# EtherealEngine/Universal-Volumetric

Hardware: AMD Instinct MI355X
Metric: frames/s encode, 100k-vert mesh + 2048^2 texture (higher is better)
Workload: dtype u8/int32 (f32 only in the quantiser)

## Files before the change

universal-volumetric_amd/csrc/geo_conn.hpp:

```cpp
__global__ void __launch_bounds__(UVOL_BLOCK) k_face_time(GeoJob *jobs) {
  JOB_OR_RETURN;
  const uint32_t i = blockIdx.x * UVOL_BLOCK + threadIdx.x;
  if (i < (uint32_t)J.nsym) { const int c = J.proc[i]; J.face_time[c / 3] = (int32_t)i; J.tstart[J.nsym - 1 - (int)i] = code_of_corner(c); }
  if (i < (uint32_t)J.ninit) { const int c = J.initc[i]; J.face_time[c / 3] = -(int32_t)i - 2; J.tstart[J.nsym + (int)i] = code_of_corner(c); }
}
__device__ __forceinline__ int att_vertex(const GeoJob &J, int slot, int c);
__device__ __forceinline__ int rec_vertex_field(const GeoJob &J, int t, int c, int r8) {
  if (r8 == 2) { const uint32_t *q = reinterpret_cast<const uint32_t *>(J.rec[1 + t]) + 4 * (size_t)(c / 3); return (int)((uint32_t)((((uint64_t)q[1] << 32) | q[0]) >> (21 * (c % 3))) & 0x1fffffu); }
  const size_t code = (size_t)code_of_corner(c);
  return r8 ? (int)((uint32_t)J.rec[1 + t][2 * code] & 0x1fffffu) : J.rec[1 + t][4 * code];
}
__global__ void __launch_bounds__(UVOL_BLOCK) k_v2d(GeoJob *jobs, int r8) {
  GeoJob &J = jobs[blockIdx.y];
  const int t = blockIdx.z;
  const uint32_t i = blockIdx.x * UVOL_BLOCK + threadIdx.x;
  const bool live = J.status == 0 && !(t > 0 && (t - 1 >= J.nad || !J.interior_seams[t - 1]));
  if (blockIdx.x * UVOL_BLOCK >= (live ? J.ne[t] : 0u)) return;
  int lo0 = 0x7fffffff, hi0 = -0x7fffffff - 1, lo1 = 0x7fffffff, hi1 = -0x7fffffff - 1;
  int iu = -1;
  if (J.qpos) for (int k = 0; k < J.nad; k++) if (J.att_kind[k] == 0 && (J.interior_seams[k] ? t == 1 + k : t == 0)) iu = k;
  if (i < J.ne[t]) {
    const int c = J.order[t][i];
    int vid, pid = 0;
    if (!J.qpos) vid = rec_vertex_field(J, t, c, r8) >> 1;
// ... 88 lines not shown
        const int v_start = act ? UVOL_ALOAD(&vval[vn_]) : 0;
        int acc = 0;
        for (int k = start; k + 1 < e; k++) {
          const int ka = (int)UVOL_READLANE(va_, k), kn = (int)UVOL_READLANE(vn_, k), kp = (int)UVOL_READLANE(vp_, k);
          const uint32_t kd = UVOL_READLANE(dpk, k);
          const int hit = (vn_ == ka ? (int)(kd & 3u) : 0) + (vn_ == kn ? (int)((kd >> 2) & 3u) : 0) + (vn_ == kp ? (int)(kd >> 4) : 0);
          acc += (int)lane > k ? hit : 0;
        }
        if (act) {
          const int av = v_start - acc;
          if (mi > 0) { const int cv = av < 2 ? 2 : (av > 7 ? 7 : av); J.ctx_of[mi] = (uint8_t)(cv - 2); }
          if (dpk & 3u) UVOL_AADD(&vval[va_], -(int)(dpk & 3u));
          UVOL_AADD(&vval[vn_], -(int)((dpk >> 2) & 3u));
          UVOL_AADD(&vval[vp_], -(int)(dpk >> 4));
        }
        UVOL_WAVE_FENCE();
        UVOL_WAVE_SYNC();
      }
      if (e < cnt) {
        const int i = base + e;
        const int lc = (int)UVOL_READLANE(c_, e);
        const int ia = (int)UVOL_READLANE(va_, e), in_ = (int)UVOL_READLANE(vn_, e), ip = (int)UVOL_READLANE(vp_, e);
        if (lane == 0) {
          const int nx = g_nxt(lc), pv = g_prv(lc);
          const int val_n = UVOL_ALOAD(&vval[in_]), val_p = UVOL_ALOAD(&vval[ip]);
          UVOL_ASTORE(&vval[in_], val_n - 1); UVOL_ASTORE(&vval[ip], val_p - 1);
          int nleft = 0, a = opp[pv];
          while (a >= 0) { if (ftime[a / 3] <= i) break; nleft++; a = opp[g_nxt(a)]; }
          UVOL_ASTORE(&vval[ia], nleft + 1);
          const int newv = nvval; int nright = 0; a = opp[nx];
          while (a >= 0) { if (ftime[a / 3] <= i) break; nright++; c2vm[g_nxt(a)] = newv; a = opp[g_prv(a)]; }
          UVOL_ASTORE(&vval[nvval], nright + 1);
          if (i > 0) { const int cv = val_n < 2 ? 2 : (val_n > 7 ? 7 : val_n); J.ctx_of[i] = (uint8_t)(cv - 2); }
        }
        nvval++;
        UVOL_WAVE_FENCE();
        UVOL_WAVE_SYNC();
        if (mi < nsym && (int)lane > e) { va_ = c2vm[c_]; vn_ = c2vm[g_nxt(c_)]; vp_ = c2vm[g_prv(c_)]; }
      }
      start = e + 1;
    }
  }
}

__global__ void __launch_bounds__(64) k_eb_ctx(GeoJob *jobs) {
  GeoJob &J = jobs[blockIdx.x];
  UVOL_SERIAL_PRIO();
  const uint32_t lane = threadIdx.x;
  const int nsym = J.status == 0 ? J.nsym : 0;
  uint32_t cnt[6] = {0, 0, 0, 0, 0, 0};
  for (int base = 1; base < nsym; base += 64) {
    const int i = base + (int)lane;
    const int cx = i < nsym ? J.ctx_of[i] : 7;
    for (int c = 0; c < 6; c++) cnt[c] += (uint32_t)__popcll(__ballot(cx == c));
  }
  uint32_t base_c[6]; { uint32_t o = 0; for (int c = 0; c < 6; c++) { base_c[c] = o; o += cnt[c]; } }
  uint32_t *all = J.ctx_all;
  const unsigned long long lt = lane == 0 ? 0ull : (~0ull >> (64 - lane));
  for (int base = 1; base < nsym; base += 64) {
    const int i = base + (int)lane;
    const bool in = i < nsym;
    const int cx = in ? J.ctx_of[i] : 7;
    const int ps = in ? J.symb[i - 1] : 0;
    const uint32_t id = ps == 0 ? 0u : (ps == 1 ? 1u : (ps == 3 ? 2u : (ps == 5 ? 3u : 4u)));
    for (int c = 0; c < 6; c++) {
      const unsigned long long m = __ballot(in && cx == c);
      if (in && cx == c) all[base_c[c] + (uint32_t)__popcll(m & lt)] = id;
      base_c[c] += (uint32_t)__popcll(m);
    }
  }
  if (lane == 0 && J.status == 0) for (int c = 0; c < 6; c++) { J.ctx_n[c] = cnt[c]; J.rs[c].n = cnt[c]; J.ctx_sym[c] = all + (base_c[c] - cnt[c]); J.rs[c].syms = J.ctx_sym[c]; }
}

__device__ __forceinline__ bool fseam_bit(const GeoJob &J, int slot, int c) { return (J.fseam[c / 3] >> (3 * slot + c % 3)) & 1u; }
__device__ __forceinline__ int st_opp(const GeoJob &J, int slot, int c) { if (c < 0) return GEO_INV; if (slot >= 0 && fseam_bit(J, slot, c)) return GEO_INV; return J.opp[c]; }
__device__ __forceinline__ int st_swl(const GeoJob &J, int slot, int c) { const int o = st_opp(J, slot, g_nxt(c)); return o < 0 ? GEO_INV : g_nxt(o); }
__device__ __forceinline__ int st_swr(const GeoJob &J, int slot, int c) { const int o = st_opp(J, slot, g_prv(c)); return o < 0 ? GEO_INV : g_prv(o); }
__device__ __forceinline__ bool vseam_bit(const GeoJob &J, int slot, uint32_t v) { return (J.vseam[slot][v >> 5] >> (v & 31)) & 1u; }
__device__ __forceinline__ int att_vertex(const GeoJob &J, int slot, int c) {
  const int v = geo_vt(J)[c];
  return (J.interior_seams[slot] && vseam_bit(J, slot, (uint32_t)v)) ? J.avert[slot][c] : v;
}
__global__ void __launch_bounds__(UVOL_BLOCK) k_seams(GeoJob *jobs) {
  JOB_OR_RETURN;
  const uint32_t f = blockIdx.x * UVOL_BLOCK + threadIdx.x;
  if (f >= J.nf) return;
  const uvol_s3 o3 = *reinterpret_cast<const uvol_s3 *>(J.opp + 3 * (size_t)f);
  const int opp_[3] = { o3.x, o3.y, o3.z };
  uint32_t bits = 0;
  for (int i = 0; i < J.nad; i++) {
    const int32_t *A = J.att_kind[i] == 0 ? J.cu : J.cn;
    const uvol_s3 a3 = *reinterpret_cast<const uvol_s3 *>(A + 3 * (size_t)f);
    const int a[3] = { a3.x, a3.y, a3.z };
    bool any = false;
    for (int k = 0; k < 3; k++) {
      uint32_t sm = 1;
      if (opp_[k] >= 0) {
        const int oo = opp_[k], fo = 3 * (oo / 3), jo = oo - fo;
        const uvol_s3 b3 = *reinterpret_cast<const uvol_s3 *>(A + fo);
        const int b[3] = { b3.x, b3.y, b3.z };
        sm = (a[(k + 1) % 3] != b[(jo + 2) % 3] || a[(k + 2) % 3] != b[(jo + 1) % 3]) ? 1u : 0u;
        if (sm) {
          any = true;
          const uint32_t va = (uint32_t)geo_vt(J)[3 * f + (k + 1) % 3], vb = (uint32_t)geo_vt(J)[3 * f + (k + 2) % 3];
          atomicOr(&J.vseam[i][va >> 5], 1u << (va & 31)); atomicOr(&J.vseam[i][vb >> 5], 1u << (vb & 31));
        }
      }
      bits |= sm << (3 * i + k);
    }
    if (any) J.interior_seams[i] = 1;
  }
  J.fseam[f] = (uint8_t)bits;
}
__global__ void __launch_bounds__(UVOL_BLOCK) k_sb_count(GeoJob *jobs) {
  JOB_OR_RETURN_UNIFORM;
  const uint32_t f = blockIdx.x * UVOL_BLOCK + threadIdx.x;
  uint32_t cnt = 0;
  if (f < J.nf) {
    const int x0 = J.tstart[f], fo = x0 >> 2, r0 = x0 & 3;
    const uvol_s3 o3 = *reinterpret_cast<const uvol_s3 *>(J.opp + 3 * (size_t)fo);
    const int opp_[3] = { o3.x, o3.y, o3.z };
    const uint32_t fs = J.fseam[fo];
    int nb[3];
    for (int k = 0; k < 3; k++) nb[k] = opp_[k] < 0 ? -1 : J.face_time[opp_[k] / 3];
    uint32_t b0 = 0, b1 = 0;
    for (int k = 0; k < 3; k++) {
      const int j = (r0 + k) % 3;
      if (opp_[j] < 0) continue;
      const int t = nb[j], df = t >= 0 ? J.nsym - 1 - t : J.nsym + (-t - 2);
      if ((uint32_t)df <= f) continue;
      b0 |= ((fs >> j) & 1u) << cnt; b1 |= ((fs >> (3 + j)) & 1u) << cnt; cnt++;
    }
    J.sbpack[f] = (uint8_t)(cnt | (b0 << 2) | (b1 << 5));
  }
  const uint32_t tot = block_sum(cnt);
  if (threadIdx.x == 0 && blockIdx.x < uvol_blocks_dev(J.nf)) J.bsum[blockIdx.x] = tot;
}
__global__ void __launch_bounds__(UVOL_BLOCK) k_sb_write(GeoJob *jobs) {
  GeoJob &J = jobs[blockIdx.y];
  const bool ok = J.status == 0;
  const uint32_t nf = ok ? J.nf : 0u, f = blockIdx.x * UVOL_BLOCK + threadIdx.x;
  const uint32_t pk = f < nf ? J.sbpack[f] : 0u, cnt = pk & 3u;
  uint32_t tot;
  const uint32_t pos = block_excl_scan(cnt, &tot) + ((ok && blockIdx.x <= uvol_blocks_dev(J.nf)) ? J.bsum[blockIdx.x] : 0);
  __shared__ uint32_t zc[2];
  if (threadIdx.x < 2) zc[threadIdx.x] = 0;
  __syncthreads();
  if (cnt) for (int i = 0; i < J.nad; i++) {
    const uint32_t b = (pk >> (2 + 3 * i)) & 7u; uint32_t z = 0;
    for (uint32_t k = 0; k < cnt; k++) { const uint8_t sb = (uint8_t)((b >> k) & 1u); J.seam_bits[i][pos + k] = sb; z += sb ? 0u : 1u; }
    if (z) atomicAdd(&zc[i], z);
  }
  __syncthreads();
  if (threadIdx.x < 2 && zc[threadIdx.x]) atomicAdd(&J.rb[1 + threadIdx.x].zeros, zc[threadIdx.x]);
  if (blockIdx.x == 0 && threadIdx.x == 0 && ok) {
    const uint32_t n = J.bsum[uvol_blocks_dev(J.nf)];
    J.n_elig = n; for (int i = 0; i < J.nad; i++) J.rb[1 + i].n = n;
  }
}

__global__ void __launch_bounds__(UVOL_BLOCK) k_aseg_a(GeoJob *jobs) {
  JOB_OR_RETURN;
  const int i = (int)blockIdx.z;
  if (i >= J.nad || !J.interior_seams[i]) return;
  const uint32_t c0 = blockIdx.x * (UVOL_BLOCK * GEO_ILP) + threadIdx.x, nc = J.nc;
  int32_t v[GEO_ILP]; uint32_t w[GEO_ILP];
#pragma unroll
  for (int k = 0; k < GEO_ILP; k++) { const uint32_t c = c0 + k * UVOL_BLOCK; v[k] = c < nc ? geo_vt(J)[c] : 0; }
#pragma unroll
  for (int k = 0; k < GEO_ILP; k++) w[k] = J.vseam[i][(uint32_t)v[k] >> 5];
#pragma unroll
  for (int k = 0; k < GEO_ILP; k++) {
    const uint32_t c = c0 + k * UVOL_BLOCK;
    if (c >= nc || !((w[k] >> ((uint32_t)v[k] & 31)) & 1u)) continue;
    if (fseam_bit(J, i, g_nxt((int)c))) J.avert[i][c] = (int32_t)(J.nverts_t[0] + atomicAdd(&J.nseg[i], 1u));
  }
}
__global__ void __launch_bounds__(UVOL_BLOCK) k_aseg_b(GeoJob *jobs) {
  JOB_OR_RETURN;
  const int i = (int)blockIdx.z;
  if (i >= J.nad || !J.interior_seams[i]) return;
  const uint32_t c0 = blockIdx.x * (UVOL_BLOCK * GEO_ILP) + threadIdx.x, nc = J.nc;
  if (c0 == 0) { const uint32_t tot = J.nverts_t[0] + J.nseg[i]; J.nverts_t[2 + i] = tot; if (tot > J.ecap) J.status = GEO_E_WS_OVERFLOW; }
  uint32_t v[GEO_ILP], w[GEO_ILP];
#pragma unroll
  for (int k = 0; k < GEO_ILP; k++) { const uint32_t c = c0 + k * UVOL_BLOCK; v[k] = c < nc ? (uint32_t)geo_vt(J)[c] : 0u; }
#pragma unroll
  for (int k = 0; k < GEO_ILP; k++) w[k] = J.vseam[i][v[k] >> 5];
#pragma unroll
  for (int k = 0; k < GEO_ILP; k++) {
    const uint32_t c = c0 + k * UVOL_BLOCK;
    if (c >= nc || !((w[k] >> (v[k] & 31)) & 1u)) continue;
    int l = (int)c; uint32_t guard = 0;
    for (;;) { const int nl = st_swl(J, i, l); if (nl < 0) break; l = nl; if (++guard > nc) { J.status = -22; return; } }
    if (l != (int)c) J.avert[i][c] = J.avert[i][l];
  }
}
```

universal-volumetric_amd/csrc/geo_walk_lds.hpp:

```cpp
__device__ __forceinline__ bool dense_table_live(const GeoJob &J, int which) { const int ai = which >= 2 ? which - 2 : 0; return !(which >= 2 && (ai >= J.nad || !J.interior_seams[ai])); }
__device__ __forceinline__ void pack_face_records(int32_t *rec, uint32_t f, const int vc[3], const int r[3], int r8) {
  if (r8 == 2) {
    uint64_t lo = 0, hi = 0;
    for (int k = 0; k < 3; k++) { lo |= (uint64_t)((uint32_t)vc[k] & 0x1fffffu) << (21 * k); hi |= (uint64_t)((uint32_t)code_of_corner(r[k]) & 0x1fffffu) << (21 * k); }
    reinterpret_cast<uint4 *>(rec)[f] = make_uint4((uint32_t)lo, (uint32_t)(lo >> 32), (uint32_t)hi, (uint32_t)(hi >> 32));
  } else if (r8) {
    uint4 *dst = reinterpret_cast<uint4 *>(rec) + 2 * (size_t)f;
    uint2 q[3];
    for (int k = 0; k < 3; k++) {
      const uint32_t R = (uint32_t)code_of_corner(r[(k + 1) % 3]) & 0x1fffffu, L = (uint32_t)code_of_corner(r[(k + 2) % 3]) & 0x1fffffu;
      q[k] = make_uint2(((uint32_t)vc[k] & 0x1fffffu) | (R << 21), (R >> 11) | (L << 10));
    }
    dst[0] = make_uint4(q[0].x, q[0].y, q[1].x, q[1].y);
    dst[1] = make_uint4(q[2].x, q[2].y, 0u, 0u);
  } else {
    int4 *dst = reinterpret_cast<int4 *>(rec) + 4 * (size_t)f;
    for (int k = 0; k < 3; k++) dst[k] = make_int4(vc[k], code_of_corner(r[(k + 1) % 3]), code_of_corner(r[(k + 2) % 3]), code_of_corner(r[k]));
    dst[3] = make_int4(0, 0, 0, 0);
  }
}
__device__ __forceinline__ void pack_dummy_record(int32_t *rec, uint32_t nf, int r8) { if (r8 == 2) reinterpret_cast<uint4 *>(rec)[nf] = make_uint4(0xffffffffu, 0xffffffffu, 0xffffffffu, 0xffffffffu); }
__global__ void __launch_bounds__(UVOL_BLOCK) k_pack_faces(GeoJob *jobs, int which, int r8) {
  JOB_OR_RETURN;
  const uint32_t f = blockIdx.x * UVOL_BLOCK + threadIdx.x;
  if (f >= J.nf) return;
  const int ai = which >= 2 ? which - 2 : 0;
  if (which >= 2 && (ai >= J.nad || !J.interior_seams[ai])) return;
  if (f == 0) pack_dummy_record(J.rec[which], J.nf, r8);
  const int32_t *opp = which == 0 ? J.opp : J.nopp;
  const uint8_t *seam = which >= 2 ? J.seam[ai] : nullptr;
  const int32_t *vert = which == 0 ? J.vert : (which == 1 ? J.bvert : J.avert[ai]);
  const uint8_t *vopen = J.vopen_d[which];
  int r[3], vc[3];
  for (int k = 0; k < 3; k++) {
    const int c = 3 * (int)f + k;
    r[k] = (seam && seam[c]) ? GEO_INV : opp[c];
    const int v = vert[c];
    vc[k] = (v << 1) | (vopen[v] ? 1 : 0);
  }
  pack_face_records(J.rec[which], f, vc, r, r8);
  if (which == 0) J.face_time[f] = -1;
}
__global__ void __launch_bounds__(UVOL_BLOCK) k_pack0(GeoJob *jobs, int r8) {
  JOB_OR_RETURN;
  const uint32_t f = blockIdx.x * UVOL_BLOCK + threadIdx.x;
  if (f == 0) { const uint32_t tot = J.n_pos + J.extra_v; J.nverts_t[0] = tot; J.nverts_t[1] = tot; if (tot > J.ecap) J.status = GEO_E_WS_OVERFLOW; }
  if (f >= J.nf) return;
  int r[3], vc[3];
  for (int k = 0; k < 3; k++) {
    const int c = 3 * (int)f + k;
    r[k] = J.opp[c];
    const uint32_t v = (uint32_t)geo_vt(J)[c];
    vc[k] = (int)((v << 1) | ((v < J.ecap && J.vopen_d[0][v]) ? 1u : 0u));
  }
  pack_face_records(J.rec[0], f, vc, r, r8);
  if (f == 0) pack_dummy_record(J.rec[0], J.nf, r8);
  J.face_time[f] = -1;
}
__global__ void __launch_bounds__(UVOL_BLOCK) k_pack_tabs(GeoJob *jobs, int r8, int first) {
  JOB_OR_RETURN;
  const int which = first + (int)blockIdx.z;
  const uint32_t f = blockIdx.x * UVOL_BLOCK + threadIdx.x;
  if (f >= J.nf || !dense_table_live(J, which)) return;
  if (f == 0) pack_dummy_record(J.rec[which], J.nf, r8);
  const int ai = which >= 2 ? which - 2 : -1;
  const uint32_t nbase = J.nverts_t[0], fs = ai >= 0 ? (uint32_t)J.fseam[f] >> (3 * ai) : 0u;
  const uvol_s3 o3 = *reinterpret_cast<const uvol_s3 *>(J.opp + 3 * (size_t)f), v3 = *reinterpret_cast<const uvol_s3 *>(geo_vt(J) + 3 * (size_t)f);
  const int oo[3] = { o3.x, o3.y, o3.z }, vv[3] = { v3.x, v3.y, v3.z };
  int r[3], vc[3];
  for (int k = 0; k < 3; k++) {
    r[k] = ((fs >> k) & 1u) ? GEO_INV : oo[k];
    uint32_t v = (uint32_t)vv[k];
    if (ai >= 0 && ((J.vseam[ai][v >> 5] >> (v & 31)) & 1u)) v = (uint32_t)J.avert[ai][3 * f + k];
    vc[k] = (int)((v << 1) | ((v >= nbase || J.vopen_d[0][v]) ? 1u : 0u));
  }
  pack_face_records(J.rec[which], f, vc, r, r8);
}

#ifdef HIPEMU
typedef int4 uvol_i4;
#else
typedef int uvol_i4 __attribute__((ext_vector_type(4)));
#endif
#ifdef HIPEMU
struct uvol_i3 { int x, y, z; };
template <typename P> __device__ __forceinline__ uvol_i3 rec3(P rec, int code) { const uvol_i4 q = rec[code]; uvol_i3 r; r.x = q.x; r.y = q.y; r.z = q.z; return r; }
#else
typedef int uvol_i3 __attribute__((ext_vector_type(3)));
template <typename P> __device__ __forceinline__ uvol_i3 rec3(P rec, int code) { return *(UVOL_G(const uvol_i3))(rec + code); }
#endif
__device__ __forceinline__ uint32_t pword(UVOL_L(uint32_t) w, int k) { return w[k]; }
#ifndef HIPEMU
__device__ __forceinline__ uint32_t pword(UVOL_G(uint32_t) w, int k) { return __hip_atomic_load(&w[k], __ATOMIC_RELAXED, __HIP_MEMORY_SCOPE_WORKGROUP); }
#endif
template <typename P> __device__ __forceinline__ bool pbit_get(P w, int i) { return (pword(w, i >> 5) >> (i & 31)) & 1u; }
template <typename P> __device__ __forceinline__ void pbit_set(P w, int i) { UVOL_OR_NORET(&w[i >> 5], 1u << (i & 31)); }
__device__ __forceinline__ int code_nxt(int x) { return (x & 3) == 2 ? x - 2 : x + 1; }
__device__ __forceinline__ int code_prv(int x) { return (x & 3) == 0 ? x + 2 : x - 1; }
__device__ __forceinline__ int corner_of_code(int x) { return 3 * (x >> 2) + (x & 3); }

#ifdef HIPEMU
struct uvol_u2 { uint32_t x, y; };
#else
typedef uint32_t uvol_u2 __attribute__((ext_vector_type(2)));
#endif
__device__ __forceinline__ void rec8_dec(uint32_t lo, uint32_t hi, int &vi, int &rc, int &lc) {
  vi = (int)(lo & 0x1fffffu);
  rc = (int)(((lo >> 21) | (hi << 11)) << 11) >> 11;
  lc = (int)(hi << 1) >> 11;
}
template <bool R8> struct RecOps;
template <> struct RecOps<false> {
  typedef UVOL_G(const uvol_i4) Ptr; typedef uvol_i3 Pre;
  static __device__ __forceinline__ Ptr ptr(const int32_t *p) { return UVOL_TO_G(const uvol_i4, reinterpret_cast<const uvol_i4 *>(p)); }
  static __device__ __forceinline__ void get(Ptr rec, int code, int &vi, int &rc, int &lc) { const uvol_i4 q = rec[code]; vi = q.x; rc = q.y; lc = q.z; }
  static __device__ __forceinline__ Pre pre(Ptr rec, int code) { return rec3(rec, code); }
  static __device__ __forceinline__ void take(const Pre &p, int &vi, int &rc, int &lc) { vi = UVOL_READFIRST(p.x); const int l_ = UVOL_READFIRST(p.z); rc = UVOL_READFIRST(p.y); lc = l_; }
};
template <> struct RecOps<true> {
  typedef UVOL_G(const uvol_u2) Ptr; typedef uvol_u2 Pre;
  static __device__ __forceinline__ Ptr ptr(const int32_t *p) { return UVOL_TO_G(const uvol_u2, reinterpret_cast<const uvol_u2 *>(p)); }
  static __device__ __forceinline__ void get(Ptr rec, int code, int &vi, int &rc, int &lc) { const uvol_u2 q = rec[code]; rec8_dec(q.x, q.y, vi, rc, lc); }
  static __device__ __forceinline__ Pre pre(Ptr rec, int code) { return rec[code]; }
  static __device__ __forceinline__ void take(const Pre &p, int &vi, int &rc, int &lc) { const uint32_t lo = (uint32_t)UVOL_READFIRST(p.x), hi = (uint32_t)UVOL_READFIRST(p.y); rec8_dec(lo, hi, vi, rc, lc); }
};

#define WALK_STG 256
#define WALK_STG_DWORDS (WALK_STG + WALK_STG / 4)
struct WalkStage {
  UVOL_L(int32_t) w; UVOL_L(uint8_t) b;
  __device__ __forceinline__ void init(UVOL_L(uint32_t) lds) { w = (UVOL_L(int32_t))lds; b = (UVOL_L(uint8_t))(lds + WALK_STG); }
  __device__ __forceinline__ void flush_words(UVOL_G(int32_t) dst, int n) {
    UVOL_G(uvol_i4) d = (UVOL_G(uvol_i4))(dst + (n - WALK_STG)); UVOL_L(const uvol_i4) s = (UVOL_L(const uvol_i4))w;
#pragma unroll 8
    for (int i = 0; i < WALK_STG / 4; i++) d[i] = s[i];
  }
  __device__ __forceinline__ void flush_bytes(UVOL_G(uint8_t) dst, int n) {
    UVOL_G(uvol_i4) d = (UVOL_G(uvol_i4))(dst + (n - WALK_STG)); UVOL_L(const uvol_i4) s = (UVOL_L(const uvol_i4))b;
#pragma unroll 8
    for (int i = 0; i < WALK_STG / 16; i++) d[i] = s[i];
  }
  __device__ __forceinline__ void tail_words(UVOL_G(int32_t) dst, int n) { for (int i = n & ~(WALK_STG - 1); i < n; i++) dst[i] = w[i & (WALK_STG - 1)]; }
  __device__ __forceinline__ void tail_bytes(UVOL_G(uint8_t) dst, int n) { for (int i = n & ~(WALK_STG - 1); i < n; i++) dst[i] = b[i & (WALK_STG - 1)]; }
};
template <bool R8, typename FB, typename VB>
__device__ __forceinline__ void eb_walk_lane0(GeoJob &J, FB fbits, VB vbits, UVOL_L(uint32_t) stg_lds) {
  typedef RecOps<R8> RO;
  const int nf = (int)J.nf;
  const typename RO::Ptr rec = RO::ptr(J.rec[0]);
  UVOL_G(int32_t) proc = UVOL_TO_G(int32_t, J.proc); UVOL_G(int32_t) stack = UVOL_TO_G(int32_t, J.stack);
  UVOL_G(int32_t) initc = UVOL_TO_G(int32_t, J.initc);
  UVOL_G(uint8_t) symb = UVOL_TO_G(uint8_t, J.symb); UVOL_G(uint8_t) start_bits = UVOL_TO_G(uint8_t, J.start_bits);
  const int dz = UVOL_LANE_ZERO();
  WalkStage stg; stg.init(stg_lds);
  int nproc = 0, ninit = 0, nstart = 0, nsplit = 0;
#define W_EMIT(SYM) do { stg.b[nproc & (WALK_STG - 1)] = (uint8_t)(SYM); nproc++; if ((nproc & (WALK_STG - 1)) == 0) { stg.flush_words(proc, nproc); stg.flush_bytes(symb, nproc); } } while (0)
  enum { T_C = 0, T_S = 1, T_L = 3, T_R = 5, T_E = 7 };
  const bool rl = J.relabel != 0; UVOL_G(const int32_t) s_of_o = UVOL_TO_G(const int32_t, J.s_of_o);
  for (int fo = 0; fo < nf; fo++) {
// ... 237 lines not shown
```

universal-volumetric_amd/csrc/geom_encode.hip:

```cpp
#include <chrono>
#include <thread>
#include "uvol_common.hpp"
#include "geom_device.hpp"
#include "uvol_ws.hpp"
#include <algorithm>
#include <map>

#define JOB_OR_RETURN GeoJob &J = jobs[blockIdx.y]; if (J.status != 0) return
#define JOB_OR_RETURN_UNIFORM GeoJob &J = jobs[blockIdx.y]; { __shared__ int job_st_; if (threadIdx.x == 0) job_st_ = J.status; __syncthreads(); if (job_st_ != 0) return; }

#include "geo_scan.hpp"
#include "geo_dedup.hpp"
#include "geo_faces.hpp"
#include "geo_corner_table.hpp"
#include "geo_walk_lds.hpp"
#include "geo_conn.hpp"
#include "geo_traverse_lds.hpp"
#include "geo_walk_simt.hpp"
#include "geo_attr.hpp"
#include "geo_matseam.hpp"
#include "geo_seq.hpp"
#include "geo_entropy.hpp"
#include "geo_layout.hpp"
struct WsItem { size_t slot, bytes; int first, last; size_t off; };
// ... 677 lines not shown
      LAUNCH(k_hp_build, dim3(he_nb_max, Ns), dim3(UVOL_BLOCK), djs);
      LAUNCH(k_edge_match, dim3(bci, Ns), dim3(UVOL_BLOCK), djs);
      LAUNCH(k_vert0, dim3(bv, Ns), dim3(UVOL_BLOCK), djs);
      LAUNCH(k_vert_fill, dim3(bc, Ns), dim3(UVOL_BLOCK), djs);
      LAUNCH(k_pack0, dim3(bf, Ns), dim3(UVOL_BLOCK), djs, fmt0);
    }
  } else {
  {
    uvol_ctx::Scope sc(ctx, "geo.k2b_faces", 0);
    const unsigned mt0 = (unsigned)((max_vals + MS_TILE - 1) / MS_TILE), mt1 = (unsigned)(((size_t)max_nfi + MS_TILE - 1) / MS_TILE);
    if (any_relabel) {
      LAUNCH(k_ms_key_pos, dim3(bv, N), dim3(UVOL_BLOCK), dj);
      LAUNCH(k_ms_count, dim3(mt0, N), dim3(UVOL_BLOCK), dj, 0);
      LAUNCH(k_ms_scan, dim3(1, N), dim3(UVOL_BLOCK), dj, 0);
      LAUNCH(k_ms_scatter, dim3(mt0, N), dim3(UVOL_BLOCK), dj, 0);
      LAUNCH(k_ms_place, dim3(ms_nb_max, N), dim3(UVOL_BLOCK), dj, 0);
    }
    LAUNCH(k_faces, dim3(bf, N), dim3(UVOL_BLOCK), dj);
    LAUNCH(k_scan_sums, dim3(1, N), dim3(UVOL_BLOCK), dj, (int)SCAN_KEEP);
    if (any_relabel) {
      LAUNCH(k_face_cidx, dim3(bf, N), dim3(UVOL_BLOCK), dj);
      LAUNCH(k_ms_count, dim3(mt1, N), dim3(UVOL_BLOCK), dj, 1);
      LAUNCH(k_ms_scan, dim3(1, N), dim3(UVOL_BLOCK), dj, 1);
      LAUNCH(k_ms_scatter, dim3(mt1, N), dim3(UVOL_BLOCK), dj, 1);
      LAUNCH(k_ms_place, dim3(ms_nb_max, N), dim3(UVOL_BLOCK), dj, 1);
      LAUNCH(k_relabel_faces, dim3(bf, N), dim3(UVOL_BLOCK), dj);
    }
    LAUNCH(k_compact_faces, dim3(bf, N), dim3(UVOL_BLOCK), dj, face_alias);
    { uvol_ctx::Scope sq(ctx, "geo.k1_quantize", algo_in); LAUNCH(k_quant_ids, dim3(bv, N, 3), dim3(UVOL_BLOCK), dj); }
  }
  {
    uvol_ctx::Scope sc(ctx, "geo.k3_corner_table", (uint64_t)n * 0 + (uint64_t)3 * max_nfi * 4 * 3);
    if (he_part_all) {
      const unsigned bt = (unsigned)(((size_t)3 * max_nfi + HE_TILE - 1) / HE_TILE);
      LAUNCH(k_hp_count, dim3(bt, N), dim3(UVOL_BLOCK), dj);
      LAUNCH(k_hp_scan, dim3(1, N), dim3(UVOL_BLOCK), dj);
      LAUNCH(k_hp_scatter, dim3(bt, N), dim3(UVOL_BLOCK), dj);
      LAUNCH(k_hp_build, dim3(he_nb_max, N), dim3(UVOL_BLOCK), dj);
    } else {
      LAUNCH(k_he_count, dim3(bci, N), dim3(UVOL_BLOCK), dj);
      LAUNCH(k_he_scan, dim3(1, N), dim3(UVOL_BLOCK), dj);
      LAUNCH(k_he_fill, dim3(bci, N), dim3(UVOL_BLOCK), dj);
    }
    LAUNCH(k_edge_match, dim3(bci, N), dim3(UVOL_BLOCK), dj);
    LAUNCH(k_vert0, dim3(bv, N), dim3(UVOL_BLOCK), dj);
    LAUNCH(k_vert_fill, dim3(bc, N), dim3(UVOL_BLOCK), dj);
  }
  }
  UVOL_HIP_CHECK(ctx, hipEventRecord(L.ev_fe, ctx->stream)); G->fe_last = L.ev_fe;
  static const int w_walk_env = [] { const char *e = getenv("UVOL_SIMT_W_WALK"); const int v = e ? atoi(e) : 0; return v < 0 ? 0 : (v > 64 ? 64 : v); }();
  static const int w_trav_env = [] { const char *e = getenv("UVOL_SIMT_W_TRAV"); const int v = e ? atoi(e) : 0; return v < 0 ? 0 : (v > 64 ? 64 : v); }();
  if (w_walk_env && wp_walk.simt_w) wp_walk.simt_w = w_walk_env;
  {
    if (!fe_sliced) LAUNCH(k_pack0, dim3(bf, N), dim3(UVOL_BLOCK), dj, fmt0);
    uvol_ctx::Scope sc(ctx, "geo.k4_eb_walk", (uint64_t)n * 32 * max_nfi);
    if (wp_walk.simt_w) {
      const unsigned W = (unsigned)wp_walk.simt_w, nb = (N + W - 1) / W;
      if (fmt0 == 2) LAUNCH(k_eb_walk_simt_f16, dim3(nb), dim3(64), dj, n, (int)W);
      else if (r8) LAUNCH((k_eb_walk_simt<true>), dim3(nb), dim3(64), dj, n, (int)W); else LAUNCH((k_eb_walk_simt<false>), dim3(nb), dim3(64), dj, n, (int)W);
    }
    else if (r8) LAUNCH_SM((k_eb_walk<true>), dim3(N), dim3(128), wp_walk.lds, dj, wp_walk.vcw, geo_walk_pf());
    else LAUNCH_SM((k_eb_walk<false>), dim3(N), dim3(128), wp_walk.lds, dj, wp_walk.vcw, geo_walk_pf());
    LAUNCH(k_face_time, dim3(bf, N), dim3(UVOL_BLOCK), dj);
  }
  {
    LAUNCH(k_eb_event_flags, dim3(bf, N), dim3(UVOL_BLOCK), dj);
    LAUNCH(k_scan_sums, dim3(1, N), dim3(UVOL_BLOCK), dj, (int)SCAN_EVENTS);
    LAUNCH(k_eb_event_compact, dim3(bf, N), dim3(UVOL_BLOCK), dj);
    LAUNCH(k_valence_init, dim3(bc, N), dim3(UVOL_BLOCK), dj);
  }
  UVOL_HIP_CHECK(ctx, hipEventRecord(L.ev_walk, ctx->stream)); G->walk_last = L.ev_walk;
  UVOL_HIP_CHECK(ctx, hipStreamWaitEvent(L.aux, L.ev_walk, 0));
  {
    { uvol_ctx::Scope sc(ctx, "geo.k4_eb_valence", 0, L.aux); LAUNCH_ON(L.aux, k_eb_valence, dim3(N), dim3(64), dj); }
    LAUNCH_ON(L.aux, k_eb_ctx, dim3(N), dim3(64), dj);
  }
  UVOL_HIP_CHECK(ctx, hipEventRecord(L.ev_val, L.aux));
  {
    uvol_ctx::Scope sc(ctx, "geo.k4b_seams", 0);
    LAUNCH(k_seams, dim3(bf, N), dim3(UVOL_BLOCK), dj);
    LAUNCH(k_sb_count, dim3(bf, N), dim3(UVOL_BLOCK), dj);
    LAUNCH(k_scan_sums, dim3(1, N), dim3(UVOL_BLOCK), dj, (int)SCAN_ELIG);
    LAUNCH(k_sb_write, dim3(bf, N), dim3(UVOL_BLOCK), dj);
    LAUNCH(k_aseg_a, dim3(bci, N, 2), dim3(UVOL_BLOCK), dj);
    LAUNCH(k_aseg_b, dim3(bci, N, 2), dim3(UVOL_BLOCK), dj);
  }
  if (!late_join) UVOL_HIP_CHECK(ctx, hipStreamWaitEvent(ctx->stream, L.ev_val, 0));
  {
    if (base_shared) LAUNCH(k_pack_tabs, dim3(bf, N, 2), dim3(UVOL_BLOCK), dj, fmtT, 2); else LAUNCH(k_pack_tabs, dim3(bf, N, 3), dim3(UVOL_BLOCK), dj, fmtT, 1);
    uvol_ctx::Scope sc(ctx, "geo.k5_traverse", (uint64_t)n * 32 * max_nfi * 3);
    if (wp_trav.simt_w > 1 && !lockstep && geo_simt_env() == 0) wp_trav.simt_w = fmtT == 2 ? ((G->blocking_call && 3u * NC <= 2048u) ? 1 : ((G->blocking_call && 3u * NC <= 4096u) ? 2 : 4)) : 1;
    if (w_trav_env && wp_trav.simt_w) wp_trav.simt_w = w_trav_env;
    launch_traversals(ctx, dj, n, wp_trav, fmtT, base_shared ? 1 : 0);
  }
  if (late_join) UVOL_HIP_CHECK(ctx, hipStreamWaitEvent(ctx->stream, L.ev_val, 0));
  { uvol_ctx::Scope sc(ctx, "geo.k5b_v2d", 0); LAUNCH(k_v2d, dim3(be, N, 3), dim3(UVOL_BLOCK), dj, fmtT); }
  {
    uvol_ctx::Scope sc(ctx, "geo.k6_predict", 0);
    if (any_mat) { LAUNCH(k_mat_vert, dim3(bc, N), dim3(UVOL_BLOCK), dj, 0); LAUNCH(k_mat_vert, dim3(bc, N), dim3(UVOL_BLOCK), dj, 1); }
    if (mat_pass) {
      uvol_ctx::Scope sm(ctx, "geo.k6b_mat_seams", 0);
      LAUNCH(k_ms_flags, dim3(bf, N), dim3(UVOL_BLOCK), dj);
      LAUNCH(k_ms_sb_count, dim3(bf, N), dim3(UVOL_BLOCK), dj);
      LAUNCH(k_scan_sums, dim3(1, N), dim3(UVOL_BLOCK), dj, (int)SCAN_ELIG);
      LAUNCH(k_ms_sb_write, dim3(bf, N), dim3(UVOL_BLOCK), dj);
      LAUNCH(k_ms_aseg, dim3(bc, N), dim3(UVOL_BLOCK), dj, 0);
      LAUNCH(k_ms_aseg, dim3(bc, N), dim3(UVOL_BLOCK), dj, 1);
      LAUNCH(k_ms_pack, dim3(bf, N), dim3(UVOL_BLOCK), dj);
      LAUNCH(k_ms_traverse, dim3(N), dim3(64), dj);
      LAUNCH(k_ms_v2d, dim3(be, N), dim3(UVOL_BLOCK), dj);
      LAUNCH(k_ms_pred, dim3(be, N), dim3(UVOL_BLOCK), dj);
    }
    LAUNCH(k_stream_setup, dim3(N), dim3(64), dj);
    LAUNCH(k_pred_pos, dim3(be, N), dim3(UVOL_BLOCK), dj);
    LAUNCH(k_pred_uv, dim3(be, N), dim3(UVOL_BLOCK), dj);
    LAUNCH(k_scan_blocks, dim3(be, N), dim3(UVOL_BLOCK), dj, (int)SCAN_ORI);
    LAUNCH(k_scan_sums, dim3(1, N), dim3(UVOL_BLOCK), dj, (int)SCAN_ORI);
    LAUNCH(k_ori_compact, dim3(be, N), dim3(UVOL_BLOCK), dj);
    LAUNCH(k_ori_bits, dim3(be, N), dim3(UVOL_BLOCK), dj);
    LAUNCH(k_face_normals, dim3(bf, N), dim3(UVOL_BLOCK), dj);
    LAUNCH(k_pred_nrm, dim3(be, N), dim3(UVOL_BLOCK), dj);
    if (any_mat) LAUNCH(k_pred_mat, dim3(be, N), dim3(UVOL_BLOCK), dj);
  }
  {
    uvol_ctx::Scope sc0(ctx, "geo.k7_hist_tables", 0);
    const unsigned NS = any_mat ? GEO_NSTREAM : GEO_NSTREAM - 1;
    LAUNCH(k_hist, dim3(uvol_blocks((size_t)9 * max_nfi, 16 * UVOL_BLOCK), NS, N), dim3(UVOL_BLOCK), dj);
    LAUNCH(k_rans_tables, dim3(NS, N), dim3(64), dj);
  }
  {
    uvol_ctx::Scope sc(ctx, "geo.k7_entropy_encode", 0);
    static const int ent_env = [] { const char *e = getenv("UVOL_ENTROPY_WAVE"); return !e ? -1 : (*e == '1' ? 1 : 0); }();
    static const int ent_w_env = [] { const char *e = getenv("UVOL_ENTROPY_W"); const int v = e ? atoi(e) : 0; return v < 0 ? 0 : (v > 64 ? 64 : v); }();
    const size_t per_frame = any_mat ? GEO_NSTREAM + GEO_NRABS : GEO_NSTREAM + GEO_NRABS - 2;
    const bool ent_wave = ent_env >= 0 ? ent_env == 1 : (ent_w_env == 0 && per_frame * NC <= (size_t)20 * G->num_cu);
    if (ent_wave) LAUNCH(k_entropy_encode, dim3(N, GEO_NSTREAM + GEO_NRABS), dim3(64), dj, uvol_debug() ? 1 : 0);
    else {
      unsigned W = 4; while (W < 64 && 5u * NC > 512u * W) W *= 2;
      if (ent_w_env) W = (unsigned)ent_w_env;
      const size_t max_alpha = std::max<size_t>(((size_t)2 << std::max(prm.q_position_attr, std::max(prm.q_texture_attr, prm.q_normal_attr))) + 8, any_mat ? 512 + 8 : 0);
      LAUNCH(k_rans_recip, dim3(uvol_blocks(max_alpha), any_mat ? GEO_NSTREAM : GEO_NSTREAM - 1, N), dim3(UVOL_BLOCK), dj);
      LAUNCH_SM(k_entropy_simt, dim3((N + W - 1) / W, GEO_NSTREAM + GEO_NRABS), dim3(64), (size_t)W * SB_STRIDE * 4, dj, n, (int)W);
    }
  }
  }
  {
    uvol_ctx::Scope sc(ctx, "geo.k8_layout_gather", 0);
    if (seq) LAUNCH(k_sq_layout, dim3(N), dim3(64), dj); else LAUNCH(k_layout, dim3(N), dim3(64), dj);
    LAUNCH(k_out_offsets, dim3(1), dim3(64), dj, n);
    LAUNCH(k_gather, dim3(64, GEO_MAXPIECES, N), dim3(UVOL_BLOCK), dj);
  }
  UVOL_HIP_CHECK(ctx, hipGetLastError());
  if (pre_up) { const int rcr = uvol_uplink_release(ctx, L.up.slot, ctx->stream); if (rcr != UVOL_OK) return rcr; }
  L.t_enq = ms_since(t_enter); L.t_enter = t_enter;
  return UVOL_OK;
}

static int geo_complete_impl(uvol_ctx *ctx, GeoLane &L) {
  static const bool timing = [] { const char *e = getenv("UVOL_TIMING"); return e && *e == '1'; }();
  auto ms_since = [](std::chrono::steady_clock::time_point a) { return std::chrono::duration<double, std::milli>(std::chrono::steady_clock::now() - a).count(); };
  const int n = L.n; const bool full = L.full, on_device = L.on_device, late_join = L.late_join;
  uint8_t *const *outs = L.outp.data(); size_t *out_lens = L.out_lens; int *status = L.status;
  const auto t_enter = L.t_enter; const double t_prep = L.t_prep, t_enq = L.t_enq;
  UVOL_HIP_CHECK(ctx, hipStreamSynchronize(ctx->stream));
  UVOL_HIP_CHECK(ctx, hipMemcpy(L.hjobs.data(), L.jobs.p, sizeof(GeoJob) * (size_t)n, hipMemcpyDeviceToHost));
  const double t_gpu = ms_since(t_enter);
  int worst = UVOL_OK;
  size_t packed = 0;
// ... 190 lines not shown
```

Baseline: 3393.

## Fold seam-vertex allocation into k_seams and swing-walk resolution into k_pack_tabs

Seam-split attribute vertex IDs are now allocated inside k_seams, using a block-level scan plus one atomicAdd per block instead of one atomic per corner. The swing-left walk that propagates IDs to corners is moved into k_pack_tabs, so the k_aseg_a and k_aseg_b launches go away. The aim is to cut two grid launches, extra passes over corners and heavy atomic contention. In exchange, k_pack_tabs now reads and writes avert while other corners may still be resolving. The ID assignment rule also changes (corner (k+2)%3 when the face edge is a seam, and a boundary check), so results could differ and races are possible.

```diff
diff --git a/universal-volumetric_amd/csrc/geo_conn.hpp b/universal-volumetric_amd/csrc/geo_conn.hpp
--- a/universal-volumetric_amd/csrc/geo_conn.hpp
+++ b/universal-volumetric_amd/csrc/geo_conn.hpp
@@ -194,35 +194,47 @@
   return (J.interior_seams[slot] && vseam_bit(J, slot, (uint32_t)v)) ? J.avert[slot][c] : v;
 }
 __global__ void __launch_bounds__(UVOL_BLOCK) k_seams(GeoJob *jobs) {
-  JOB_OR_RETURN;
+  JOB_OR_RETURN_UNIFORM;
   const uint32_t f = blockIdx.x * UVOL_BLOCK + threadIdx.x;
-  if (f >= J.nf) return;
-  const uvol_s3 o3 = *reinterpret_cast<const uvol_s3 *>(J.opp + 3 * (size_t)f);
-  const int opp_[3] = { o3.x, o3.y, o3.z };
-  uint32_t bits = 0;
-  for (int i = 0; i < J.nad; i++) {
-    const int32_t *A = J.att_kind[i] == 0 ? J.cu : J.cn;
-    const uvol_s3 a3 = *reinterpret_cast<const uvol_s3 *>(A + 3 * (size_t)f);
-    const int a[3] = { a3.x, a3.y, a3.z };
-    bool any = false;
-    for (int k = 0; k < 3; k++) {
-      uint32_t sm = 1;
-      if (opp_[k] >= 0) {
-        const int oo = opp_[k], fo = 3 * (oo / 3), jo = oo - fo;
-        const uvol_s3 b3 = *reinterpret_cast<const uvol_s3 *>(A + fo);
-        const int b[3] = { b3.x, b3.y, b3.z };
-        sm = (a[(k + 1) % 3] != b[(jo + 2) % 3] || a[(k + 2) % 3] != b[(jo + 1) % 3]) ? 1u : 0u;
-        if (sm) {
-          any = true;
-          const uint32_t va = (uint32_t)geo_vt(J)[3 * f + (k + 1) % 3], vb = (uint32_t)geo_vt(J)[3 * f + (k + 2) % 3];
-          atomicOr(&J.vseam[i][va >> 5], 1u << (va & 31)); atomicOr(&J.vseam[i][vb >> 5], 1u << (vb & 31));
+  const int nad = J.nad;
+  uint32_t bits = 0, inner = 0;
+  if (f < J.nf) {
+    const uvol_s3 o3 = *reinterpret_cast<const uvol_s3 *>(J.opp + 3 * (size_t)f);
+    const int opp_[3] = { o3.x, o3.y, o3.z };
+    for (int i = 0; i < nad; i++) {
+      const int32_t *A = J.att_kind[i] == 0 ? J.cu : J.cn;
+      const uvol_s3 a3 = *reinterpret_cast<const uvol_s3 *>(A + 3 * (size_t)f);
+      const int a[3] = { a3.x, a3.y, a3.z };
+      for (int k = 0; k < 3; k++) {
+        uint32_t sm = 1;
+        if (opp_[k] >= 0) {
+          const int oo = opp_[k], fo = 3 * (oo / 3), jo = oo - fo;
+          const uvol_s3 b3 = *reinterpret_cast<const uvol_s3 *>(A + fo);
+          const int b[3] = { b3.x, b3.y, b3.z };
+          sm = (a[(k + 1) % 3] != b[(jo + 2) % 3] || a[(k + 2) % 3] != b[(jo + 1) % 3]) ? 1u : 0u;
+          if (sm) {
+            inner |= 1u << (3 * i + k);
+            const uint32_t va = (uint32_t)geo_vt(J)[3 * f + (k + 1) % 3], vb = (uint32_t)geo_vt(J)[3 * f + (k + 2) % 3];
+            atomicOr(&J.vseam[i][va >> 5], 1u << (va & 31)); atomicOr(&J.vseam[i][vb >> 5], 1u << (vb & 31));
+          }
         }
+        bits |= sm << (3 * i + k);
       }
-      bits |= sm << (3 * i + k);
-    }
-    if (any) J.interior_seams[i] = 1;
-  }
-  J.fseam[f] = (uint8_t)bits;
+      if ((inner >> (3 * i)) & 7u) J.interior_seams[i] = 1;
+    }
+    J.fseam[f] = (uint8_t)bits;
+  }
+  __shared__ uint32_t seg0[2];
+  for (int i = 0; i < nad; i++) {
+    const uint32_t m = (inner >> (3 * i)) & 7u;
+    uint32_t tot;
+    const uint32_t ex = block_excl_scan((uint32_t)__popc(m), &tot);
+    if (tot == 0) continue;
+    if (threadIdx.x == 0) seg0[i] = J.nverts_t[0] + atomicAdd(&J.nseg[i], tot);
+    __syncthreads();
+    uint32_t id = seg0[i] + ex;
+    for (int k = 0; k < 3; k++) if ((m >> k) & 1u) J.avert[i][3 * f + (k + 2) % 3] = (int32_t)id++;
+  }
 }
 __global__ void __launch_bounds__(UVOL_BLOCK) k_sb_count(GeoJob *jobs) {
   JOB_OR_RETURN_UNIFORM;
@@ -271,40 +283,29 @@
   }
 }
 
-__global__ void __launch_bounds__(UVOL_BLOCK) k_aseg_a(GeoJob *jobs) {
+__global__ void __launch_bounds__(UVOL_BLOCK) k_pack_tabs(GeoJob *jobs, int r8, int first) {
   JOB_OR_RETURN;
-  const int i = (int)blockIdx.z;
-  if (i >= J.nad || !J.interior_seams[i]) return;
-  const uint32_t c0 = blockIdx.x * (UVOL_BLOCK * GEO_ILP) + threadIdx.x, nc = J.nc;
-  int32_t v[GEO_ILP]; uint32_t w[GEO_ILP];
-#pragma unroll
-  for (int k = 0; k < GEO_ILP; k++) { const uint32_t c = c0 + k * UVOL_BLOCK; v[k] = c < nc ? geo_vt(J)[c] : 0; }
-#pragma unroll
-  for (int k = 0; k < GEO_ILP; k++) w[k] = J.vseam[i][(uint32_t)v[k] >> 5];
-#pragma unroll
-  for (int k = 0; k < GEO_ILP; k++) {
-    const uint32_t c = c0 + k * UVOL_BLOCK;
-    if (c >= nc || !((w[k] >> ((uint32_t)v[k] & 31)) & 1u)) continue;
-    if (fseam_bit(J, i, g_nxt((int)c))) J.avert[i][c] = (int32_t)(J.nverts_t[0] + atomicAdd(&J.nseg[i], 1u));
-  }
-}
-__global__ void __launch_bounds__(UVOL_BLOCK) k_aseg_b(GeoJob *jobs) {
-  JOB_OR_RETURN;
-  const int i = (int)blockIdx.z;
-  if (i >= J.nad || !J.interior_seams[i]) return;
-  const uint32_t c0 = blockIdx.x * (UVOL_BLOCK * GEO_ILP) + threadIdx.x, nc = J.nc;
-  if (c0 == 0) { const uint32_t tot = J.nverts_t[0] + J.nseg[i]; J.nverts_t[2 + i] = tot; if (tot > J.ecap) J.status = GEO_E_WS_OVERFLOW; }
-  uint32_t v[GEO_ILP], w[GEO_ILP];
-#pragma unroll
-  for (int k = 0; k < GEO_ILP; k++) { const uint32_t c = c0 + k * UVOL_BLOCK; v[k] = c < nc ? (uint32_t)geo_vt(J)[c] : 0u; }
-#pragma unroll
-  for (int k = 0; k < GEO_ILP; k++) w[k] = J.vseam[i][v[k] >> 5];
-#pragma unroll
-  for (int k = 0; k < GEO_ILP; k++) {
-    const uint32_t c = c0 + k * UVOL_BLOCK;
-    if (c >= nc || !((w[k] >> (v[k] & 31)) & 1u)) continue;
-    int l = (int)c; uint32_t guard = 0;
-    for (;;) { const int nl = st_swl(J, i, l); if (nl < 0) break; l = nl; if (++guard > nc) { J.status = -22; return; } }
-    if (l != (int)c) J.avert[i][c] = J.avert[i][l];
-  }
-}
+  const int which = first + (int)blockIdx.z;
+  const uint32_t f = blockIdx.x * UVOL_BLOCK + threadIdx.x;
+  if (f >= J.nf || !dense_table_live(J, which)) return;
+  if (f == 0) pack_dummy_record(J.rec[which], J.nf, r8);
+  const int ai = which >= 2 ? which - 2 : -1;
+  const uint32_t nbase = J.nverts_t[0], fs = ai >= 0 ? (uint32_t)J.fseam[f] >> (3 * ai) : 0u;
+  if (f == 0 && ai >= 0) { const uint32_t tot = nbase + J.nseg[ai]; J.nverts_t[2 + ai] = tot; if (tot > J.ecap) J.status = GEO_E_WS_OVERFLOW; }
+  const uvol_s3 o3 = *reinterpret_cast<const uvol_s3 *>(J.opp + 3 * (size_t)f), v3 = *reinterpret_cast<const uvol_s3 *>(geo_vt(J) + 3 * (size_t)f);
+  const int oo[3] = { o3.x, o3.y, o3.z }, vv[3] = { v3.x, v3.y, v3.z };
+  int r[3], vc[3];
+  for (int k = 0; k < 3; k++) {
+    r[k] = ((fs >> k) & 1u) ? GEO_INV : oo[k];
+    uint32_t v = (uint32_t)vv[k];
+    if (ai >= 0 && ((J.vseam[ai][v >> 5] >> (v & 31)) & 1u)) {
+      const int c = 3 * (int)f + k; int l = c; uint32_t guard = 0;
+      for (;;) { const int nl = st_swl(J, ai, l); if (nl < 0) break; l = nl; if (++guard > J.nc) { J.status = -22; return; } }
+      const bool bnd = J.opp[g_nxt(l)] < 0;
+      if (!bnd) v = (uint32_t)J.avert[ai][l];
+      if (bnd || l != c) J.avert[ai][c] = (int32_t)v;
+    }
+    vc[k] = (int)((v << 1) | ((v >= nbase || J.vopen_d[0][v]) ? 1u : 0u));
+  }
+  pack_face_records(J.rec[which], f, vc, r, r8);
+}
diff --git a/universal-volumetric_amd/csrc/geo_walk_lds.hpp b/universal-volumetric_amd/csrc/geo_walk_lds.hpp
--- a/universal-volumetric_amd/csrc/geo_walk_lds.hpp
+++ b/universal-volumetric_amd/csrc/geo_walk_lds.hpp
@@ -56,25 +56,6 @@
   pack_face_records(J.rec[0], f, vc, r, r8);
   if (f == 0) pack_dummy_record(J.rec[0], J.nf, r8);
   J.face_time[f] = -1;
-}
-__global__ void __launch_bounds__(UVOL_BLOCK) k_pack_tabs(GeoJob *jobs, int r8, int first) {
-  JOB_OR_RETURN;
-  const int which = first + (int)blockIdx.z;
-  const uint32_t f = blockIdx.x * UVOL_BLOCK + threadIdx.x;
-  if (f >= J.nf || !dense_table_live(J, which)) return;
-  if (f == 0) pack_dummy_record(J.rec[which], J.nf, r8);
-  const int ai = which >= 2 ? which - 2 : -1;
-  const uint32_t nbase = J.nverts_t[0], fs = ai >= 0 ? (uint32_t)J.fseam[f] >> (3 * ai) : 0u;
-  const uvol_s3 o3 = *reinterpret_cast<const uvol_s3 *>(J.opp + 3 * (size_t)f), v3 = *reinterpret_cast<const uvol_s3 *>(geo_vt(J) + 3 * (size_t)f);
-  const int oo[3] = { o3.x, o3.y, o3.z }, vv[3] = { v3.x, v3.y, v3.z };
-  int r[3], vc[3];
-  for (int k = 0; k < 3; k++) {
-    r[k] = ((fs >> k) & 1u) ? GEO_INV : oo[k];
-    uint32_t v = (uint32_t)vv[k];
-    if (ai >= 0 && ((J.vseam[ai][v >> 5] >> (v & 31)) & 1u)) v = (uint32_t)J.avert[ai][3 * f + k];
-    vc[k] = (int)((v << 1) | ((v >= nbase || J.vopen_d[0][v]) ? 1u : 0u));
-  }
-  pack_face_records(J.rec[which], f, vc, r, r8);
 }
 
 #ifdef HIPEMU
diff --git a/universal-volumetric_amd/csrc/geom_encode.hip b/universal-volumetric_amd/csrc/geom_encode.hip
--- a/universal-volumetric_amd/csrc/geom_encode.hip
+++ b/universal-volumetric_amd/csrc/geom_encode.hip
@@ -783,8 +783,6 @@
     LAUNCH(k_sb_count, dim3(bf, N), dim3(UVOL_BLOCK), dj);
     LAUNCH(k_scan_sums, dim3(1, N), dim3(UVOL_BLOCK), dj, (int)SCAN_ELIG);
     LAUNCH(k_sb_write, dim3(bf, N), dim3(UVOL_BLOCK), dj);
-    LAUNCH(k_aseg_a, dim3(bci, N, 2), dim3(UVOL_BLOCK), dj);
-    LAUNCH(k_aseg_b, dim3(bci, N, 2), dim3(UVOL_BLOCK), dj);
   }
   if (!late_join) UVOL_HIP_CHECK(ctx, hipStreamWaitEvent(ctx->stream, L.ev_val, 0));
   {
```

After: 3438 (median of 2 runs). Within noise of the previous version (+1.3%).
